# JiQi-da/Mixed-Graph-ADMM

Hardware: AMD Instinct MI355X
Metric: ADMM iters/sec x batch (sample-iterations/s) (higher is better)
Workload: dtype f32; 1 GPU; cfg2: PEMS04-shaped synthetic graph N=307 (path+chords, 340 edges), kNN k=4, T=24, t_in=12; batch_per_gpu=4096, global_batch=4096, ablation=None, graph=kNN-directed, max_cg_iter=100, parallelism=batch-sharded x1, no collective on the convergence path, final RCCL gather, all_finite=True

## Files before the change

mixed-graph-admm_amd/csrc/engine.h:

```cpp
#pragma once
#include <math.h>
#include <cmath>
#include <stdlib.h>
#include <string.h>

#include <algorithm>
#include <type_traits>

#include "common.h"
#include "cldr_tiles.h"
#include "stream_kernels.h"
#include "lds_args.h"
#include "lds_banks.h"

namespace {

struct LhsDef {
    int kind;
    int hth;
    double c1, c2;
};

enum VecId {
    V_XA, V_XB, V_ZUA, V_ZUB, V_ZDA, V_ZDB, V_PHIA, V_PHIB, V_GAM, V_GU, V_GD, V_Y, V_MASK,
    V_R, V_P, V_Q, V_AP, V_RHS, V_TMP, V_IO0, V_IO1, V_COUNT
};

constexpr int LAG = 2;
constexpr int NRED_MAX = 6;
constexpr int PROF_POOL = 32768;
constexpr int LDS_SETS = 3;
constexpr int LDS_NBOUND = 4;
constexpr int LDS_MAXJ_POOL = LDS_MAXJ;
constexpr int NACT_LOG = 1 << 16;

template <typename S>
// ... 21 lines not shown
    int* h_flag = nullptr;
    hipEvent_t ev_ring[LAG + 1] = {nullptr};
    int want_blocks = 2048;
    struct TileMetaDev { int R = 0; int GW = 0; int* tl_col = nullptr; float* tl_w = nullptr; int* halo = nullptr; int* h_rowptr = nullptr; int* h_col = nullptr; float* h_val = nullptr; };
    TileMetaDev tmeta[3];
    struct CldrDev {
        int state = 0, NT = 0;
        int *n0 = nullptr, *nC = nullptr, *rows = nullptr, *dcol = nullptr, *dcnt = nullptr, *tcol = nullptr, *tcnt = nullptr;
        float *dw = nullptr, *tw = nullptr;
    } cldr_dev;
    int use_fused = 1;
    int use_fold = 1;
    int use_fold_lu = 1;
    int sweep_rev = 1;
    int cldr_tile_major = 1;
    int cur_P = 0;
    int use_tile = 1;
    int64_t ws_bytes = 0;
    struct LdsPlan {
        bool ok = false;
        int G = 0, TPG = 0, TS = 0, nthreads = 0, block = 0, NR = 0, csr_ints = 0, maxt = 1024, sb = 0, uniform45 = 0, slots = 0;
        int tail_pairs = 0, lds_img0 = 0, lds_img_ints = 0;
        int off_rp_u = 0, off_rp_d = 0, off_en_u = 0, off_en_d = 0, off_lead_t = 0, off_tail_t = 0, off_diag = 0;
        size_t lds_bytes = 0;
    } lds;
    int* d_lds_csr = nullptr;
    double* d_m2 = nullptr;
    int lds_async = 1;
    int* d_stop = nullptr;
    double* d_ps_ring = nullptr;
    int* d_pstop = nullptr;
    double* d_ps_full = nullptr;
    size_t ps_full_elems = 0;
    int sp_B = 0;
    std::vector<double> sp_val[6];
    LdsSampleParams* d_sp = nullptr;
    std::vector<float*> lds_ring_extra;
    int64_t lds_instance = -1;
    int lds_chunk = LDS_MAXJ_POOL;
    hipStream_t st_side = nullptr;
    hipEvent_t ev_main[LDS_NBOUND] = {nullptr}, ev_side[LDS_NBOUND] = {nullptr};
    bool prof_on = false;
    std::vector<hipEvent_t> prof_ev;
    std::vector<int> prof_tag;
    std::vector<double> prof_lb;
    std::vector<int> prof_ref;
// ... 1299 lines not shown
        lds.maxt = (best == 12 && lds.block <= 640) ? 640 : 1024;
        lds.sb = (sb_env && ((best == 12 && lds.maxt == 640) || best == 8)) ? 1 : 0;
        const int NR = N + (lds.block - lds.nthreads);
        lds.NR = NR;
        lds.uniform45 = (!band && (best == 8 || best == 12) && !lds.sb && !getenv("MGADMM_LDS_RAGGED")) ? 1 : 0;
        for (int i = 0; i < N && lds.uniform45; ++i) {
            int ndiag = 0;
            for (int e = g->hWd.rowptr[i]; e < g->hWd.rowptr[i + 1]; ++e) ndiag += g->hWd.col[e] == i;
            if (g->hWu.rowptr[i + 1] - g->hWu.rowptr[i] != 4 || g->hWd.rowptr[i + 1] - g->hWd.rowptr[i] != 5 || ndiag != 1) lds.uniform45 = 0;
        }
        std::vector<float> diag_d(NR, 0.f), diag_t(NR, 0.f);
        auto strip_diag = [&](const HostCsr& h, std::vector<float>& dg) {
            HostCsr o;
            o.rowptr.push_back(0);
            for (int i = 0; i < N; ++i) {
                for (int e = h.rowptr[i]; e < h.rowptr[i + 1]; ++e) {
                    if (h.col[e] == i) dg[i] += h.val[e];
                    else { o.col.push_back(h.col[e]); o.val.push_back(h.val[e]); }
                }
                o.rowptr.push_back((int)o.col.size());
            }
            return o;
        };
        const HostCsr hWdT_off = band ? HostCsr() : strip_diag(g->hWdT, diag_t);
        int maxlen_t = 0;
        if (!band)
            for (int i = 0; i < N; ++i) maxlen_t = std::max(maxlen_t, hWdT_off.rowptr[i + 1] - hWdT_off.rowptr[i]);
        const int tp = band ? 0 : (std::max(0, maxlen_t - LDS_NLEAD) + 1) / 2;
        const int WT = LDS_NLEAD + 2 * tp;
        lds.tail_pairs = tp;
        const HostCsr hWd_tab = band ? HostCsr() : (lds.uniform45 ? strip_diag(g->hWd, diag_d) : g->hWd);
        auto with_ghosts = [&](const HostCsr& h, int fixed_len) {
            HostCsr o;
            o.rowptr.assign(h.rowptr.begin(), h.rowptr.begin() + N + 1);
            o.col = h.col; o.val = h.val;
            for (int r = N; r < NR; ++r) {
                for (int e = 0; e < fixed_len; ++e) { o.col.push_back(r); o.val.push_back(0.f); }
                o.rowptr.push_back((int)o.col.size());
            }
            return o;
        };
        const HostCsr hu = with_ghosts(g->hWu, lds.uniform45 ? 4 : 0);
        const HostCsr hd = band ? HostCsr() : with_ghosts(hWd_tab, lds.uniform45 ? 4 : 0);
        const int nu = hu.nnz(), nd = band ? 0 : hd.nnz();
        auto al4 = [](int v) { return (v + 3) & ~3; };
        int off = 0;
        lds.off_rp_u = off; off += NR + 1;
        lds.off_rp_d = off; off += NR + 1;
        off = al4(off);
        lds.off_en_u = off; off += 2 * nu;
        lds.off_en_d = off; off += 2 * nd;
        lds.off_lead_t = off; off += 2 * NR * LDS_NLEAD;
        off = al4(off);
        lds.off_tail_t = off; off += 2 * NR * 2 * tp + 4;
        const int tail_ints = off - lds.off_tail_t;
        lds.off_diag = off; off += 2 * NR;
        off += 8;
        lds.csr_ints = off;
        lds.lds_img0 = lds.uniform45 ? lds.off_tail_t : 0;
        lds.lds_img_ints = lds.uniform45 ? tail_ints : lds.off_diag;
        int ts = (T + 3) / 4 * 4;
        if (((ts / 4) & 1) == 0) ts += 4;
        auto bytes_for = [&](int stride, int slots) {
            const size_t LN = (size_t)NR * stride;
            return sizeof(float) * ((lds.sb ? 1 : 2) * LN + ((4 - (LN & 3)) & 3) + 32 + 16 * 12 + (size_t)slots * 2 * lds.block * best)
                   + sizeof(int) * (size_t)lds.lds_img_ints;
        };
        if (bytes_for(ts, 0) > 160 * 1024) ts = T;
        lds.TS = ts;
        if (bytes_for(ts, 0) > 160 * 1024) { lds = LdsPlan(); return MGADMM_OK; }
        lds.slots = (lds.uniform45 && !getenv("MGADMM_LDS_NOSLOTS") && bytes_for(ts, 1) <= 160 * 1024) ? 1 : 0;
        lds.lds_bytes = bytes_for(ts, lds.slots);
        std::vector<int> img(off, 0);
        const bool bank_order = !band && best % 4 == 0 && ((lds.TS / 4) & 1) && !getenv("MGADMM_LDS_TABLE_ORDER");
        long search_steps = 4000;
        if (const char* e = getenv("MGADMM_LDS_BANK_SEARCH")) search_steps = atol(e);
        auto slot_order = [&](const HostCsr& h, ldsbank::Stream stream) {
            std::vector<int> order(h.nnz());
            for (int e = 0; e < h.nnz(); ++e) order[e] = e;
            if (!bank_order || h.nnz() == 0) return order;
// ... 9 lines not shown
                std::vector<int> pos(N);
                for (int i = 0; i < N; ++i) pos[i] = i;
                const ldsbank::Result r = ldsbank::improve_targeted(q, m, pos, search_steps);
                if (getenv("MGADMM_LDS_BANK_STATS"))
                    fprintf(stderr, "[mgadmm] lds bank search: stream %d, %d entries: %.0f -> %.0f conflict cycles per application (%ld steps)\n",
                            (int)stream, h.rowptr[N], r.before, r.after, r.moves);
            }
            for (int e = 0; e < h.rowptr[N]; ++e) order[e] = m.src[e];
            return order;
        };
        auto put_entry = [&](int at, int col, float w) {
            img[at] = col * lds.TS;
            memcpy(&img[at + 1], &w, 4);
        };
        auto put_csr = [&](const HostCsr& h, int off_rp, int off_en, ldsbank::Stream stream) {
            const std::vector<int> order = slot_order(h, stream);
            for (int i = 0; i <= NR; ++i) img[off_rp + i] = h.rowptr[i];
            for (int e = 0; e < h.nnz(); ++e) put_entry(off_en + 2 * e, h.col[order[e]], h.val[order[e]]);
        };
        const ldsbank::Stream fixed_or_pairs = lds.uniform45 ? ldsbank::FIXED : ldsbank::PAIRS;
        put_csr(hu, lds.off_rp_u, lds.off_en_u, fixed_or_pairs);
        if (!band) {
            put_csr(hd, lds.off_rp_d, lds.off_en_d, fixed_or_pairs);
            HostCsr ht;
            ht.rowptr.push_back(0);
            std::vector<int> from;
            for (int i = 0; i < N; ++i) {
                const int e0 = hWdT_off.rowptr[i], len = hWdT_off.rowptr[i + 1] - e0;
                for (int e = 0; e < WT; ++e) {
                    ht.col.push_back(e < len ? hWdT_off.col[e0 + e] : i);
                    ht.val.push_back(e < len ? hWdT_off.val[e0 + e] : 0.f);
                    from.push_back(e < len ? e0 + e : -1);
                }
                ht.rowptr.push_back((int)ht.col.size());
            }
            const std::vector<int> order = slot_order(ht, ldsbank::FIXED);
            for (int r = 0; r < NR; ++r)
                for (int e = 0; e < WT; ++e) {
                    const int at = e < LDS_NLEAD ? lds.off_lead_t + 2 * (r * LDS_NLEAD + e)
                                                 : lds.off_tail_t + 2 * (r * 2 * tp + (e - LDS_NLEAD));
                    if (r < N) put_entry(at, ht.col[order[r * WT + e]], ht.val[order[r * WT + e]]);
                    else put_entry(at, r, 0.f);
                }
            put_entry(lds.off_tail_t + 2 * NR * 2 * tp, 0, 0.f);
            put_entry(lds.off_tail_t + 2 * NR * 2 * tp + 2, 0, 0.f);
            memcpy(&img[lds.off_diag], diag_d.data(), sizeof(float) * NR);
            memcpy(&img[lds.off_diag + NR], diag_t.data(), sizeof(float) * NR);
        }
        MG_HIP(hipMalloc(&d_lds_csr, sizeof(int) * off));
        MG_HIP(hipMemcpy(d_lds_csr, img.data(), sizeof(int) * off, hipMemcpyHostToDevice));
        MG_HIP(hipMalloc(&d_m2, sizeof(double) * T * N * (1 + (size_t)(Bmax + 63) / 64)));
        MG_HIP(hipMalloc(&d_stop, sizeof(int)));
        MG_HIP(hipMemset(d_stop, 0, sizeof(int)));
        MG_HIP(hipMalloc(&d_ps_ring, sizeof(double) * LDS_SETS * LDS_MAXJ_POOL * MGADMM_NMETRIC * Bp_max));
        MG_HIP(hipMalloc(&d_pstop, sizeof(int) * (2 * (size_t)Bp_max + 1)));
        {
            int lo = 0, hi = 0;
            MG_HIP(hipDeviceGetStreamPriorityRange(&lo, &hi));
            if (const char* e = getenv("MGADMM_LDS_SIDE_PRIO")) lo = atoi(e) > 0 ? hi : lo;
            MG_HIP(hipStreamCreateWithPriority(&st_side, hipStreamNonBlocking, lo));
            for (auto& e : ev_main) MG_HIP(hipEventCreateWithFlags(&e, hipEventDisableTiming));
            for (auto& e : ev_side) MG_HIP(hipEventCreateWithFlags(&e, hipEventDisableTiming));
        }
        lds.ok = true;
        return MGADMM_OK;
    }

    int launch_lds(const LdsArgs& a, int B) {
        const bool timed = prof_open(0, 0.0);
        LdsLaunch L{lds.TPG, lds.maxt, lds.sb, lds.uniform45, lds.slots, lds.block, lds.lds_bytes, &lds_instance};
        const int rc = mg_lds_iteration(L, a, B, st);
        if (timed) prof_close();
        return rc;
    }

    int solve_lds(const void* y, const void* mask, int B, const void* x0, const mgadmm_state* state_in, void* x_out,
                  const mgadmm_state* state_out, mgadmm_history* hist) {
        if constexpr (!std::is_same<S, float>::value) {
            return MGADMM_ERR_UNSUPPORTED;
        } else {
            const int abl = p.ablation;
            const bool has_phi = (abl == MGADMM_ABL_NONE || abl == MGADMM_ABL_DGLR);
            const bool has_zd = (abl != MGADMM_ABL_DGLR);
            const int max_it = p.max_admm_iter;
            const bool record = p.record_cg_coeffs && hist && hist->cg_alpha && hist->cg_beta;
            const int Bp = (B + 63) / 64 * 64;
            const size_t TN = (size_t)T * N;
            if (hist && hist->metrics_per_sample) {
                size_t need = (size_t)max_it * MGADMM_NMETRIC * B;
// ... 26 lines not shown
            constexpr int NRING = (int)(sizeof(ring_ids) / sizeof(ring_ids[0]));
            const int J = sched == CHUNKS ? std::max(1, std::min(std::min(lds_chunk, LDS_MAXJ_POOL), max_it)) : 1;
            {
                const int need = LDS_SETS * (J - 1) + LDS_NBOUND - NRING;
                while ((int)lds_ring_extra.size() < need) {
                    float* b = nullptr;
                    MG_HIP(hipMalloc(&b, vec_elems * sizeof(S)));
                    lds_ring_extra.push_back(b);
                    ws_bytes += (int64_t)(vec_elems * sizeof(S));
                }
            }
            auto ring = [&](int j) -> float* { return j < NRING ? (float*)vec[ring_ids[j]] : lds_ring_extra[j - NRING]; };
            auto xbuf = [&](int k) -> float* {
                if (k == max_it) return xo_;
                if (sched != CHUNKS) return ring(k & 1);
                if (k % J == 0) return ring((k / J) % LDS_NBOUND);
                return ring(LDS_NBOUND + ((k / J) % LDS_SETS) * (J - 1) + (k % J - 1));
            };
            float *zu = vec[V_ZUA], *zd = vec[V_ZDA], *phi = vec[V_PHIA], *gam = vec[V_GAM], *gu = vec[V_GU], *gd = vec[V_GD];
            if (state_in) {
                const size_t nb = (size_t)B * TN * sizeof(float);
                if (x0 != nullptr && xbuf(0) != x0) MG_HIP(hipMemcpyAsync(xbuf(0), x0, nb, hipMemcpyDeviceToDevice, st));
                auto in = [&](float* dst, const void* src) {
                    return src == nullptr ? (int)MGADMM_OK : mg_lds_state_layout(true, T, N, lds.TPG, B, (const float*)src, dst, st);
                };
                MG_TRY(in(zu, state_in->zu));
                MG_TRY(in(gu, state_in->gamma_u));
                MG_TRY(in(zd, state_in->zd));
                MG_TRY(in(gd, state_in->gamma_d));
                MG_TRY(in(phi, state_in->phi));
                MG_TRY(in(gam, state_in->gamma));
            } else {
                float tm = 0, t2m = 0;
                for (int t = 0; t < p.t_in; ++t) { tm += (float)t; t2m += (float)t * (float)t; }
                tm /= (float)p.t_in;
                t2m /= (float)p.t_in;
                const float den = t2m - tm * tm;
                MG_TRY(mg_lds_init(mask != nullptr, T, p.t_in, N, lds.TPG, B, tm, den, (const float*)y, (const float*)mask, xbuf(0), zu, zd, gam, gu, gd,
                                   d_nonfinite, st));
            }
            LdsArgs a{};
            a.T = T; a.N = N; a.TN = (int)TN; a.TS = lds.TS; a.t_in = p.t_in; a.G = lds.G; a.B = B; a.Bp = Bp;
            a.nthreads = lds.nthreads; a.NR = lds.NR; a.tail_pairs = lds.tail_pairs;
            a.has_phi = has_phi; a.has_zd = has_zd;
            const LhsDef dx = lhs_def(MGADMM_LHS_X);
            a.lhsx_kind = dx.kind == 1 ? 1 : 0;
            a.cx1 = (float)dx.c1; a.cx2 = (float)dx.c2;
            a.band = g->mode == MGADMM_TEMPORAL_BAND; a.skip = g->skip;
            a.q1 = a.band ? 0 : g->q1;
            a.max_cg = p.max_cg_iter; a.record = record ? 1 : 0;
            a.rho = (float)p.rho; a.rho_u = (float)p.rho_u; a.rho_d = (float)p.rho_d;
            a.mu_u = (float)p.mu_u; a.mu_d1 = (float)p.mu_d1; a.mu_d2 = (float)p.mu_d2;
            a.cg_tol2 = p.cg_tol * p.cg_tol;
            a.csr = d_lds_csr; a.lds_img0 = lds.lds_img0; a.lds_img_ints = lds.lds_img_ints;
            a.off_rp_u = lds.off_rp_u; a.off_rp_d = lds.off_rp_d;
            a.off_en_u = lds.off_en_u; a.off_en_d = lds.off_en_d; a.off_lead_t = lds.off_lead_t; a.off_tail_t = lds.off_tail_t; a.off_diag = lds.off_diag;
            a.band_w = g->band_w;
            a.zu = zu; a.zd = zd; a.phi = phi; a.gam = gam; a.gu = gu; a.gd = gd;
            {
                const int ncu = dev_cus > 0 ? dev_cus : 256;
                int us = 48;
                if (const char* e = getenv("MGADMM_LDS_STAGGER_US")) us = atoi(e);
                a.stagger_wgs = ncu;
                a.stagger_ticks = (B >= 2 * ncu && us > 0) ? us * 100 : 0;
            }
            a.y = (const float*)y; a.mask = (const float*)mask;
            a.alpha_hist = record ? (float*)d_alpha_hist : nullptr; a.beta_hist = record ? (float*)d_beta_hist : nullptr;
            a.nonfinite = d_nonfinite;
            a.stop = sched == DEVSTOP ? d_stop : nullptr;
            if (sched == DEVSTOP) MG_HIP(hipMemsetAsync(d_stop, 0, sizeof(int), st));
            if (sched == CHUNKS && !ps_mode) MG_HIP(hipMemsetAsync(d_ps_ring, 0, sizeof(double) * LDS_SETS * J * MGADMM_NMETRIC * Bp, st));
            int* const d_pcount = d_pstop + Bp_max;
            if (ps_mode) {
                a.pstop = d_pstop; a.pstop_count = d_pcount; a.x_final = xo_; a.admm_tol = p.admm_tol;
            }
            if (sp_B > 0) a.sp = d_sp;
            auto all_stopped = [&](int c, bool* done) -> int {
                MG_HIP(hipMemcpyAsync(h_flag + 1 + c % (LAG + 1), d_pcount, sizeof(int), hipMemcpyDeviceToHost, st));
                MG_HIP(hipEventRecord(ev_ring[c % (LAG + 1)], st));
// ... 95 lines not shown
            }
            if (sched == DEVSTOP) {
                MG_HIP(hipMemcpyAsync(h_flag + 1, d_stop, sizeof(int), hipMemcpyDeviceToHost, st));
                MG_HIP(hipStreamSynchronize(st));
                const int sw = h_flag[1];
                if (sw > 0) n_done = sw;
                else if (sw < 0) { n_done = -sw; rc_final = MGADMM_ERR_NONFINITE; }
            }
            std::vector<int> nps;
            if (ps_mode) {
                int* const d_nps = d_pstop + Bp_max + 1;
                MG_TRY(mg_lds_ps_history(d_ps_full, d_pstop, n_done, max_it, B, Bp, d_nps, d_hist,
                                         (hist && hist->metrics_per_sample) ? d_hist_ps : nullptr, st));
                nps.resize(B);
                MG_HIP(hipMemcpyAsync(nps.data(), d_nps, sizeof(int) * B, hipMemcpyDeviceToHost, st));
                MG_HIP(hipStreamSynchronize(st));
                n_done = *std::max_element(nps.begin(), nps.end());
            }
            float* const xc = ps_mode ? xo_ : xbuf(n_done);
            if (xc != xo_)
                MG_HIP(hipMemcpyAsync(x_out, xc, (size_t)B * TN * sizeof(float), hipMemcpyDeviceToDevice, st));
            if (state_out) {
                auto out = [&](void* dst, const float* src) {
                    return dst == nullptr ? (int)MGADMM_OK : mg_lds_state_layout(false, T, N, lds.TPG, B, src, (float*)dst, st);
                };
                MG_TRY(out(state_out->zu, zu));
                MG_TRY(out(state_out->zd, zd));
                if (has_phi) {
                    MG_TRY(out(state_out->phi, phi));
                    MG_TRY(out(state_out->gamma, gam));
                }
                MG_TRY(out(state_out->gamma_u, gu));
                MG_TRY(out(state_out->gamma_d, gd));
            }
            return finish_history(hist, n_done, B, Bp, rc_final, ps_mode ? nps.data() : nullptr);
        }
    }

    int finish_history(mgadmm_history* hist, int n_done, int B, int Bp, int rc_final, const int* nps = nullptr) {
        if (hist) {
            hist->n_iters = n_done;
            if (hist->n_iters_per_sample)
                for (int b = 0; b < B; ++b) hist->n_iters_per_sample[b] = nps ? nps[b] : n_done;
            if (hist->metrics)
                MG_HIP(hipMemcpyAsync(hist->metrics, d_hist, sizeof(double) * (size_t)n_done * MGADMM_NMETRIC, hipMemcpyDeviceToHost, st));
            if (hist->delta_x_per_step && !nps)
                MG_HIP(hipMemcpyAsync(hist->delta_x_per_step, d_dxps, sizeof(double) * (size_t)n_done * T, hipMemcpyDeviceToHost, st));
// ... 33 lines not shown
```

mixed-graph-admm_amd/csrc/lds_args.h:

```cpp
#pragma once
#include <hip/hip_runtime.h>

constexpr int LDS_NLEAD = 5;
constexpr int LDS_MAXJ = 16;

struct LdsArgsCore {
    int T, N, TN, TS, t_in, G, B, Bp;
    int nthreads;
    int NR;
    int has_phi, has_zd, first;
    int J;
    int lhsx_kind;
    int band, skip, q1;
    int max_cg;
    int record;
    int stagger_wgs, stagger_ticks;
    int tail_pairs;
    float rho, rho_u, rho_d, mu_u, mu_d1, mu_d2;
    float cx1, cx2;
    double cg_tol2;
    const int* csr;
    int lds_img0, lds_img_ints;
    int off_rp_u, off_rp_d, off_en_u, off_en_d, off_lead_t, off_tail_t;
    int off_diag;
    const float* band_w;
    float *zu, *zd, *phi, *gam, *gu, *gd;
    const float* y;
    const float* mask;
    double* ps;
    int* cg_iters;
    float* alpha_hist;
    float* beta_hist;
    int* nonfinite;
    const int* stop;
};
struct LdsSampleParams {
    float rho, rho_u, rho_d, mu_u, mu_d1, mu_d2;
    float cx1, cx2;
};
struct LdsArgs : LdsArgsCore {
    float* xs[LDS_MAXJ + 1];
    int* pstop;
    int* pstop_count;
    float* x_final;
    double admm_tol;
    int it0;
    const LdsSampleParams* sp;
};

struct LdsLaunch {
    int tpg;
    int maxt;
    int sb;
    int uniform45;
    int slots;
    int block;
    size_t lds_bytes;
    int64_t* instance;
};

int mg_lds_iteration(const LdsLaunch& L, const LdsArgs& a, int B, hipStream_t st);
int mg_lds_iteration_ps(const LdsLaunch& L, const LdsArgs& a, int B, hipStream_t st);
int mg_lds_iteration_pp(const LdsLaunch& L, const LdsArgs& a, int B, hipStream_t st);
int mg_lds_init(bool masked, int T, int t_in, int N, int TPG, int B, float tm, float den, const float* y, const float* mask, float* x,
                float* zu, float* zd, float* gam, float* gu, float* gd, int* nonfinite, hipStream_t st);
int mg_lds_state_layout(bool to_thread_major, int T, int N, int TPG, int B, const float* src, float* dst, hipStream_t st);
int mg_lds_dxps(int T, int N, int B, const float* x, const float* xo, double* scratch, double* out, const int* stop, hipStream_t st);
int mg_lds_ps_history(const double* ps, const int* pstop, int n_it, int max_it, int B, int Bp, int* n_per_sample, double* metrics,
                      double* out_ps, hipStream_t st);
int mg_lds_stop_test(const double* metrics_row, const int* nonfinite, int has_phi, int has_zd, double tol, int it, int* stop, hipStream_t st);
```

mixed-graph-admm_amd/csrc/lds_kernels.h:

```cpp
#pragma once
#include "common.h"
#include "lds_args.h"



template <int CTRL, int ROW_MASK>
__device__ __forceinline__ float dpp_step(float v) {
    const int moved = __builtin_amdgcn_update_dpp(0, __float_as_int(v), CTRL, ROW_MASK, 0xf, false);
    return v + __int_as_float(moved);
}
__device__ __forceinline__ float wave_sum(float v) {
    v = dpp_step<0x111, 0xf>(v);
    v = dpp_step<0x112, 0xf>(v);
    v = dpp_step<0x114, 0xf>(v);
    v = dpp_step<0x118, 0xf>(v);
    asm("s_nop 1\n\tv_add_f32_dpp %0, %0, %0 row_bcast:15 row_mask:0xa bank_mask:0xf\n\t"
        "s_nop 1\n\tv_add_f32_dpp %0, %0, %0 row_bcast:31 row_mask:0xc bank_mask:0xf\n\ts_nop 1" : "+v"(v));
    return __int_as_float(__builtin_amdgcn_readlane(__float_as_int(v), 63));
}

struct BlockRed {
    float* red;
    int par;
    int lane, wave, nwaves;
// ... 187 lines not shown
        for (int k = 0; k < TPG; ++k) v[k] = p[k];
    }
}

__device__ __forceinline__ float rhs_half(float rho, float z, float g) { return __builtin_fmaf(rho, z, -g) * 0.5f; }
__device__ __forceinline__ float ldrt_operand(float rho, float phi, float gam) { return __builtin_fmaf(rho, phi, gam); }

template <int TPG, bool BAND, int NU = 0, int ND = 0, int TP = -1>
struct LdsCtx {
    int T, TS, N, t0, i, ig;
    bool active;
    float* P;
    float* Q;
    const i2v* en_u; const i2v* en_d;
    const i2v* lead_t;
    const i2v* tail_t;
    int u0, u1, d0, d1;
    int tail_pairs;
    unsigned so0;
    unsigned kN4[TPG];
    f2 wdiag;
    int skip, q1;
    const float* band_w;

    __device__ __forceinline__ unsigned glb0() const { return 4u * (unsigned)(t0 * N + ig); }
    __device__ __forceinline__ int own() const { return i * TS + t0; }

    static constexpr bool UNI = NU > 0 && ND > 0;
    static constexpr int NDO = ND > 0 ? ND - 1 : 0;
    struct Rows {
        i2v u[NU > 0 ? NU : 1];
        i2v d[NDO > 0 ? NDO : 1];
        i2v t[LDS_NLEAD];
    };
    __device__ __forceinline__ i2v reg_entry(i2v e, const float* IMG) const {
        i2v r;
        r.x = lds_addr(IMG) + 4 * (e.x + t0);
        r.y = e.y;
        return r;
    }
    template <int NE>
    __device__ __forceinline__ void load_rows(const i2v* EN, int e0, const float* IMG, i2v (&en)[NE]) const {
        i2v raw[NE];
#pragma unroll
        for (int u = 0; u < NE; ++u) raw[u] = EN[e0 + u];
#pragma unroll
        for (int u = 0; u < NE; ++u) en[u] = reg_entry(raw[u], IMG);
    }

    template <int NE>
    __device__ __forceinline__ void gather_regs(const i2v (&en)[NE], int delta, float (&acc)[TPG]) const {
#pragma unroll
// ... 10 lines not shown
            wacc<TPG>(en[NE - 1], va, acc);
        }
    }
    __device__ __forceinline__ void gather(const float* SRC, const i2v* EN, int e0, int e1, float (&acc)[TPG]) const {
        const float* base = SRC + t0;
        i2v na = EN[e0], nb = EN[e0 + 1];
        int e = e0;
        for (; e + 1 < e1; e += 2) {
            const i2v ea = na, eb = nb;
            float va[TPG], vb[TPG];
            lds_load<TPG>(base + ea.x, va);
            lds_load<TPG>(base + eb.x, vb);
            na = EN[e + 2];
            nb = EN[e + 3];
            wacc<TPG>(ea, va, acc);
            wacc<TPG>(eb, vb, acc);
        }
        if (e < e1) {
            float va[TPG];
            lds_load<TPG>(base + na.x, va);
            wacc<TPG>(na, va, acc);
        }
    }
    __device__ __forceinline__ void gather_tail(const float* SRC, float (&acc)[TPG]) const {
        const float* base = SRC + t0;
        if constexpr (TP >= 0) {
            const lds_i4* row = reinterpret_cast<const lds_i4*>(tail_t + (size_t)i * 2 * TP);
            lds_i4 e2[TP > 0 ? TP : 1];
#pragma unroll
            for (int j = 0; j < TP; ++j) e2[j] = row[j];
#pragma unroll
            for (int j = 0; j < TP; ++j) {
                float va[TPG], vb[TPG];
                lds_load<TPG>(base + e2[j].x, va);
                lds_load<TPG>(base + e2[j].z, vb);
                wacc<TPG>(e2[j].xy, va, acc);
                wacc<TPG>(e2[j].zw, vb, acc);
            }
        } else {
            const lds_i4* row = reinterpret_cast<const lds_i4*>(tail_t + (size_t)i * 2 * tail_pairs);
            lds_i4 nxt = row[0];
            for (int j = 0; j < tail_pairs; ++j) {
                const lds_i4 e2 = nxt;
                float va[TPG], vb[TPG];
                lds_load<TPG>(base + e2.x, va);
                lds_load<TPG>(base + e2.z, vb);
                nxt = row[j + 1];
                wacc<TPG>(e2.xy, va, acc);
                wacc<TPG>(e2.zw, vb, acc);
            }
        }
    }

    __device__ __forceinline__ void mul_wu(const float* SRC, float (&acc)[TPG], const Rows& R) const {
#pragma unroll
        for (int k = 0; k < TPG; ++k) acc[k] = 0.f;
        if constexpr (UNI) gather_regs<NU>(R.u, lds_addr(SRC) - lds_addr(P), acc);
        else gather(SRC, en_u, u0, u1, acc);
    }
    __device__ __forceinline__ void mul_wd(const float* SRC, float (&acc)[TPG], const Rows& R, const float* own_run = nullptr) const {
// ... 368 lines not shown
    float xc[TPG], vc[TPG];
#pragma unroll
    for (int k = 0; k < TPG; ++k) xc[k] = vc[k] = 0.f;
    for (int trip = 0; trip < J; ++trip) {
#if defined(__HIP_DEVICE_COMPILE__)
    asm volatile("" : "+s"(kp));
    asm volatile("" : "+v"(tid));
    asm volatile("" : "+s"(b));
    const LdsArgs __attribute__((address_space(4)))& a = *kp;
#else
    const LdsArgs& a = *kp;
#endif
    const bool first = a.first && trip == 0;
#ifdef MGADMM_PHASE_CLOCK
    unsigned long long stamps[MGADMM_NMETRIC];
#define MG_STAMP(m) do { asm volatile("s_waitcnt vmcnt(0) lgkmcnt(0)" ::: "memory"); stamps[m] = wall_clock64(); } while (0)
#else
#define MG_STAMP(m) do { } while (0)
#endif
    MG_STAMP(0);
    LdsCtx<TPG, BAND, NU, ND, TP> c;
    c.T = a.T; c.TS = a.TS; c.N = a.N;
    c.active = tid < a.nthreads;
    {
        const int g = c.active ? tid / a.N : 0;
        c.ig = c.active ? tid - g * a.N : 0;
        c.i = c.active ? c.ig : a.N + (tid - a.nthreads);
        c.t0 = g * TPG;
    }
    c.P = P; c.Q = Q;
    c.skip = a.skip; c.q1 = a.q1; c.band_w = a.band_w;
    c.tail_pairs = a.tail_pairs;
#pragma unroll
    for (int k = 0; k < TPG; ++k) { c.kN4[k] = 4u * (unsigned)k * (unsigned)a.N; MG_PIN_S(c.kN4[k]); }
    c.so0 = c.active ? 4u * TPG * (unsigned)tid : 0u;
    {
        const int* tab = ENTG ? a.csr : img - a.lds_img0;
        c.en_u = reinterpret_cast<const i2v*>(tab + a.off_en_u);
        c.en_d = reinterpret_cast<const i2v*>(tab + a.off_en_d);
        c.lead_t = reinterpret_cast<const i2v*>(tab + a.off_lead_t);
        c.tail_t = reinterpret_cast<const i2v*>(img - a.lds_img0 + a.off_tail_t);
    }
    c.wdiag = mk2(0.f, 0.f);
    if constexpr (!BAND) {
        const float* dg = reinterpret_cast<const float*>(a.csr + a.off_diag);
        c.wdiag = mk2(dg[c.i], dg[a.NR + c.i]);
    }
    constexpr bool UNI = NU > 0 && ND > 0;
    constexpr int NDO = ND > 0 ? ND - 1 : 0;
    typename LdsCtx<TPG, BAND, NU, ND, TP>::Rows R;
    auto fetch_u = [&]() {
        if constexpr (UNI) {
// ... 106 lines not shown
    }
    MG_STAMP(1);
    __syncthreads();
    c.u0 = c.u1 = c.d0 = c.d1 = 0;
    if constexpr (NU > 0) c.u0 = c.i * NU;
    else { c.u0 = img[a.off_rp_u - a.lds_img0 + c.i]; c.u1 = img[a.off_rp_u - a.lds_img0 + c.i + 1]; }
    if constexpr (!BAND) {
        if constexpr (ND > 0) c.d0 = c.i * NDO;
        else { c.d0 = img[a.off_rp_d - a.lds_img0 + c.i]; c.d1 = img[a.off_rp_d - a.lds_img0 + c.i + 1]; }
    }
    BlockRed br;
    br.red = red; br.par = 0; br.lane = tid & 63; br.wave = tid >> 6; br.nwaves = (nthr + 63) >> 6;
    auto mput = [&](int m, float val) {
        const float w = wave_sum(val);
        if (br.lane == 0) mred[br.wave * NMRED + m] = w;
    };

    auto refresh = [&]() {
        MG_PIN_V(tid);
        MG_PIN_V(c.i); MG_PIN_V(c.ig); MG_PIN_V(c.t0);
        c.active = tid < a.nthreads;
        c.so0 = c.active ? 4u * TPG * (unsigned)tid : 0u;
        br.lane = tid & 63; br.wave = tid >> 6;
    };

    if (has_phi && first) {
        float ph[TPG];
        c.template put<-1>(P, x);
        __syncthreads();
        c.op_ldr(P, x, ph, R);
        c.puts(phi, ph);
        float gq[TPG];
        request1s(gam, gq);
#pragma unroll
        for (int k = 0; k < TPG; ++k) v[k] = c.active ? ldrt_operand(rho, ph[k], gq[k]) : 0.f;
        __syncthreads();
    }
    fetch_d();

    float rhs[TPG];
    {
        float l[TPG];
#pragma unroll
        for (int k = 0; k < TPG; ++k) l[k] = 0.f;
        if (has_phi) {
            c.template put<+1>(P, v);
// ... 270 lines not shown
        };
        double pri = rnorm(MGADMM_M_PRI_ZU), dual = rnorm(MGADMM_M_DUAL_ZU);
        if (has_phi) { pri = fmax(pri, rnorm(MGADMM_M_PRI_PHI)); dual = fmax(dual, rnorm(MGADMM_M_DUAL_PHI)); }
        if (has_zd) { pri = fmax(pri, rnorm(MGADMM_M_PRI_ZD)); dual = fmax(dual, rnorm(MGADMM_M_DUAL_ZD)); }
        const double atol = a.admm_tol;
        if (pri < atol && dual < atol) {
            c.putg(a.x_final + sb, xc);
            if (tid == 0) {
                a.pstop[b] = a.it0 + trip + 1;
                atomicAdd(a.pstop_count, 1);
            }
            break;
        }
    }
    }
}

__host__ __device__ __forceinline__ int lds_state_index(int t, int i, int N, int TPG) { return ((t / TPG) * N + i) * TPG + t % TPG; }

template <bool MASKED>
__global__ __launch_bounds__(256) void k_init_lds(int T, int t_in, int N, int TPG, int B, float tm, float den, const float* __restrict__ y,
                                                  const float* __restrict__ mask, float* __restrict__ x, float* __restrict__ zu,
                                                  float* __restrict__ zd, float* __restrict__ gam, float* __restrict__ gu,
                                                  float* __restrict__ gd, int* __restrict__ nonfinite) {
#pragma clang fp contract(off)
    const int i = blockIdx.x * 256 + threadIdx.x;
    const int b = blockIdx.y;
    if (i >= N) return;
    const size_t sb = (size_t)b * T * N;
    float w, c0;
    const float* yb = MASKED ? y + sb : y + (size_t)b * t_in * N;
    const float* mb = MASKED ? mask + sb : nullptr;
    if (!MASKED) {
        float sy = 0.f, sty = 0.f;
        for (int t = 0; t < t_in; ++t) {
            const float v = yb[t * N + i];
            sy += v;
            sty += (float)t * v;
        }
        const float ym = sy / (float)t_in;
        w = (sty / (float)t_in - tm * ym) / den;
        c0 = ym - w * tm;
    } else {
        float n = 0, ts = 0, t2s = 0, ys = 0, tys = 0;
        for (int t = 0; t < T; ++t) {
            const float m = mb[t * N + i], v = yb[t * N + i];
            n += m; ts += (float)t * m; t2s += (float)(t * t) * m;
            ys += v * m; tys += (float)t * v * m;
        }
        const float tmean = ts / n, t2mean = t2s / n, ymean = ys / n, tymean = tys / n;
        float tm2 = tmean * tmean;
        asm volatile("" : "+v"(tm2));
        const float dn = t2mean - tm2;
        w = (tymean - tmean * ymean) / dn;
        c0 = ymean - w * tmean;
        if (!(fabsf(w) <= 3.0e38f) || !(fabsf(c0) <= 3.0e38f)) *nonfinite = 1;
    }
    auto value = [&](int t) {
        if (!MASKED) return (t < t_in) ? yb[t * N + i] : w * (float)t + c0;
        return (w * (float)t + c0) * (1.f - mb[t * N + i]) + yb[t * N + i];
    };
    for (int t0 = 0; t0 < T; t0 += TPG) {
        const size_t es = sb + (size_t)((t0 / TPG) * N + i) * TPG;
        if (TPG % 4 == 0) {
            for (int k = 0; k < TPG; k += 4) {
                lds_f4 q;
                q.x = value(t0 + k); q.y = value(t0 + k + 1); q.z = value(t0 + k + 2); q.w = value(t0 + k + 3);
                x[sb + (size_t)(t0 + k) * N + i] = q.x; x[sb + (size_t)(t0 + k + 1) * N + i] = q.y;
                x[sb + (size_t)(t0 + k + 2) * N + i] = q.z; x[sb + (size_t)(t0 + k + 3) * N + i] = q.w;
                *reinterpret_cast<lds_f4*>(zu + es + k) = q;
                *reinterpret_cast<lds_f4*>(zd + es + k) = q;
                lds_f4 c; c.x = c.y = c.z = c.w = 0.1f;
                *reinterpret_cast<lds_f4*>(gam + es + k) = c;
                *reinterpret_cast<lds_f4*>(gu + es + k) = c;
                *reinterpret_cast<lds_f4*>(gd + es + k) = c;
            }
        } else {
            for (int k = 0; k < TPG; ++k) {
                const float v = value(t0 + k);
                x[sb + (size_t)(t0 + k) * N + i] = v;
                zu[es + k] = v; zd[es + k] = v;
                gam[es + k] = 0.1f; gu[es + k] = 0.1f; gd[es + k] = 0.1f;
            }
        }
    }
}

template <bool TO_THREAD_MAJOR>
__global__ __launch_bounds__(256) void k_state_layout(int T, int N, int TPG, const float* __restrict__ src, float* __restrict__ dst) {
    const int e = blockIdx.x * 256 + threadIdx.x;
    if (e >= T * N) return;
    const size_t sb = (size_t)blockIdx.y * T * N;
    const int t = e / N, i = e - t * N;
    const int es = lds_state_index(t, i, N, TPG);
    if (TO_THREAD_MAJOR) dst[sb + es] = src[sb + e];
    else dst[sb + e] = src[sb + es];
}

static __global__ __launch_bounds__(256) void k_dxps_sm(int TN, int B, const float* __restrict__ x, const float* __restrict__ xo,
                                                 double* __restrict__ part, const int* __restrict__ stop) {
    const int e = blockIdx.x * 256 + threadIdx.x;
    if (e >= TN || (stop != nullptr && *stop != 0)) return;
    const int b0 = blockIdx.y * 64, b1 = min(B, b0 + 64);
    double s = 0.0;
    for (int b = b0; b < b1; ++b) s += (double)x[(size_t)b * TN + e] - (double)xo[(size_t)b * TN + e];
    part[(size_t)blockIdx.y * TN + e] = s;
}

static __global__ __launch_bounds__(64) void k_dxps_sm4(int TN, int B, const float* __restrict__ x, const float* __restrict__ xo,
                                                 double* __restrict__ part, const int* __restrict__ stop) {
    const int e = (blockIdx.x * 64 + threadIdx.x) * 4;
    if (e >= TN || (stop != nullptr && *stop != 0)) return;
    const int b0 = blockIdx.y * 64, b1 = min(B, b0 + 64);
    double s0 = 0.0, s1 = 0.0, s2 = 0.0, s3 = 0.0;
    int b = b0;
    for (; b + 4 <= b1; b += 4) {
        lds_f4 a[4], o[4];
// ... 100 lines not shown
```

mixed-graph-admm_amd/csrc/lds_launch.hip:

```cpp
#include "lds_dispatch.h"

int mg_lds_iteration(const LdsLaunch& L, const LdsArgs& a, int B, hipStream_t st) {
    if (a.sp != nullptr) return mg_lds_iteration_pp(L, a, B, st);
    return a.pstop != nullptr ? mg_lds_iteration_ps(L, a, B, st) : lds_dispatch(L, a, B, st);
}

int mg_lds_init(bool masked, int T, int t_in, int N, int TPG, int B, float tm, float den, const float* y, const float* mask, float* x,
                float* zu, float* zd, float* gam, float* gu, float* gd, int* nonfinite, hipStream_t st) {
    dim3 grid((N + 255) / 256, B);
    if (masked) hipLaunchKernelGGL((k_init_lds<true>), grid, dim3(256), 0, st, T, t_in, N, TPG, B, tm, den, y, mask, x, zu, zd, gam, gu, gd, nonfinite);
    else hipLaunchKernelGGL((k_init_lds<false>), grid, dim3(256), 0, st, T, t_in, N, TPG, B, tm, den, y, (const float*)nullptr, x, zu, zd, gam, gu, gd, nonfinite);
    MG_HIP(hipGetLastError());
    return MGADMM_OK;
}

int mg_lds_state_layout(bool to_thread_major, int T, int N, int TPG, int B, const float* src, float* dst, hipStream_t st) {
    dim3 grid((T * N + 255) / 256, B);
    if (to_thread_major) hipLaunchKernelGGL((k_state_layout<true>), grid, dim3(256), 0, st, T, N, TPG, src, dst);
    else hipLaunchKernelGGL((k_state_layout<false>), grid, dim3(256), 0, st, T, N, TPG, src, dst);
    MG_HIP(hipGetLastError());
    return MGADMM_OK;
}

int mg_lds_dxps(int T, int N, int B, const float* x, const float* xo, double* scratch, double* out, const int* stop, hipStream_t st) {
    const int TN = T * N, nsl = (B + 63) / 64;
    if (TN % 4 == 0 && ((uintptr_t)x % 16) == 0 && ((uintptr_t)xo % 16) == 0)
        hipLaunchKernelGGL(k_dxps_sm4, dim3((TN / 4 + 63) / 64, nsl), dim3(64), 0, st, TN, B, x, xo, scratch + TN, stop);
    else
        hipLaunchKernelGGL(k_dxps_sm, dim3((TN + 255) / 256, nsl), dim3(256), 0, st, TN, B, x, xo, scratch + TN, stop);
    hipLaunchKernelGGL(k_dxps_sm_mean, dim3((TN + 255) / 256), dim3(256), 0, st, TN, B, nsl, (const double*)(scratch + TN), scratch, stop);
    hipLaunchKernelGGL(k_dxps_sm_final, dim3(T), dim3(256), 0, st, T, N, (const double*)scratch, out, stop);
    MG_HIP(hipGetLastError());
    return MGADMM_OK;
}

int mg_lds_stop_test(const double* metrics_row, const int* nonfinite, int has_phi, int has_zd, double tol, int it, int* stop, hipStream_t st) {
    hipLaunchKernelGGL(k_lds_stop_test, dim3(1), dim3(64), 0, st, metrics_row, nonfinite, has_phi, has_zd, tol, it, stop);
    MG_HIP(hipGetLastError());
    return MGADMM_OK;
}

int mg_lds_ps_history(const double* ps, const int* pstop, int n_it, int max_it, int B, int Bp, int* n_per_sample, double* metrics,
// ... 6 lines not shown
```

Measured before the change: 2.848 million ADMM sample-iterations/s.

## Reorder graph rows by transpose tail class so waves skip empty tail pairs

Relabels graph nodes so rows are sorted by how many transposed-directed-graph tail pairs they need, and records a per-wave maximum degree packed into a 64-bit launch word. In the LDS kernel each wave reads its count and runs only the tail-pair gathers its rows need, instead of the worst-case count for every row. Init and state-layout kernels are updated to map nodes to the permuted rows, and the bank-conflict table ordering is rebuilt for the padded-per-limit table. The cost is an extra indirection for the thread's node index, more wave-uniform branching, and more code for the relabeled layout.

```diff
diff --git a/mixed-graph-admm_amd/csrc/engine.h b/mixed-graph-admm_amd/csrc/engine.h
--- a/mixed-graph-admm_amd/csrc/engine.h
+++ b/mixed-graph-admm_amd/csrc/engine.h
@@ -12,6 +12,7 @@
 #include "stream_kernels.h"
 #include "lds_args.h"
 #include "lds_banks.h"
+#include "lds_rows.h"
 
 namespace {
 
@@ -79,6 +80,9 @@
         int G = 0, TPG = 0, TS = 0, nthreads = 0, block = 0, NR = 0, csr_ints = 0, maxt = 1024, sb = 0, uniform45 = 0, slots = 0;
         int tail_pairs = 0, lds_img0 = 0, lds_img_ints = 0;
         int off_rp_u = 0, off_rp_d = 0, off_en_u = 0, off_en_d = 0, off_lead_t = 0, off_tail_t = 0, off_diag = 0;
+        int row_order = 0;
+        int off_node = 0, off_rown = 0;
+        uint64_t npos_word = 0;
         size_t lds_bytes = 0;
     } lds;
     int* d_lds_csr = nullptr;
@@ -1424,14 +1428,27 @@
             }
             return o;
         };
-        const HostCsr hWdT_off = band ? HostCsr() : strip_diag(g->hWdT, diag_t);
-        int maxlen_t = 0;
+        std::vector<int> deg_t(N, 0);
         if (!band)
-            for (int i = 0; i < N; ++i) maxlen_t = std::max(maxlen_t, hWdT_off.rowptr[i + 1] - hWdT_off.rowptr[i]);
+            for (int i = 0; i < N; ++i)
+                for (int e = g->hWdT.rowptr[i]; e < g->hWdT.rowptr[i + 1]; ++e) deg_t[i] += g->hWdT.col[e] != i;
+        const int maxlen_t = N > 0 ? *std::max_element(deg_t.begin(), deg_t.end()) : 0;
         const int tp = band ? 0 : (std::max(0, maxlen_t - LDS_NLEAD) + 1) / 2;
         const int WT = LDS_NLEAD + 2 * tp;
         lds.tail_pairs = tp;
-        const HostCsr hWd_tab = band ? HostCsr() : (lds.uniform45 ? strip_diag(g->hWd, diag_d) : g->hWd);
+        const char* ro_env = getenv("MGADMM_LDS_ROW_ORDER");
+        lds.row_order = (lds.uniform45 && tp <= 3) ? (ro_env ? std::max(0, std::min(atoi(ro_env), 2)) : (int)ldsrows::TAIL_CLASS) : 0;
+        const ldsrows::Plan rows = ldsrows::make_plan(deg_t, lds.G, WT, lds.row_order, LDS_NLEAD);
+        lds.npos_word = 0;
+        if (lds.uniform45 && tp <= 3 && !ldsrows::pack_npos(rows, &lds.npos_word)) {
+            mg_set_error("lds: row plan does not fit its launch word (%d waves)", (int)rows.npos.size());
+            return MGADMM_ERR_INVALID;
+        }
+        const HostCsr Wu = lds.row_order ? ldsrows::relabel(g->hWu, rows) : g->hWu;
+        const HostCsr Wd = lds.row_order ? ldsrows::relabel(g->hWd, rows) : g->hWd;
+        const HostCsr WdT = lds.row_order ? ldsrows::relabel(g->hWdT, rows) : g->hWdT;
+        const HostCsr hWdT_off = band ? HostCsr() : strip_diag(WdT, diag_t);
+        const HostCsr hWd_tab = band ? HostCsr() : (lds.uniform45 ? strip_diag(Wd, diag_d) : Wd);
         auto with_ghosts = [&](const HostCsr& h, int fixed_len) {
             HostCsr o;
             o.rowptr.assign(h.rowptr.begin(), h.rowptr.begin() + N + 1);
@@ -1442,7 +1459,7 @@
             }
             return o;
         };
-        const HostCsr hu = with_ghosts(g->hWu, lds.uniform45 ? 4 : 0);
+        const HostCsr hu = with_ghosts(Wu, lds.uniform45 ? 4 : 0);
         const HostCsr hd = band ? HostCsr() : with_ghosts(hWd_tab, lds.uniform45 ? 4 : 0);
         const int nu = hu.nnz(), nd = band ? 0 : hd.nnz();
         auto al4 = [](int v) { return (v + 3) & ~3; };
@@ -1458,6 +1475,8 @@
         const int tail_ints = off - lds.off_tail_t;
         lds.off_diag = off; off += 2 * NR;
         off += 8;
+        lds.off_node = off; off += NR;
+        lds.off_rown = off; off += N;
         lds.csr_ints = off;
         lds.lds_img0 = lds.uniform45 ? lds.off_tail_t : 0;
         lds.lds_img_ints = lds.uniform45 ? tail_ints : lds.off_diag;
@@ -1513,24 +1532,18 @@
         put_csr(hu, lds.off_rp_u, lds.off_en_u, fixed_or_pairs);
         if (!band) {
             put_csr(hd, lds.off_rp_d, lds.off_en_d, fixed_or_pairs);
-            HostCsr ht;
-            ht.rowptr.push_back(0);
-            std::vector<int> from;
-            for (int i = 0; i < N; ++i) {
-                const int e0 = hWdT_off.rowptr[i], len = hWdT_off.rowptr[i + 1] - e0;
-                for (int e = 0; e < WT; ++e) {
-                    ht.col.push_back(e < len ? hWdT_off.col[e0 + e] : i);
-                    ht.val.push_back(e < len ? hWdT_off.val[e0 + e] : 0.f);
-                    from.push_back(e < len ? e0 + e : -1);
-                }
-                ht.rowptr.push_back((int)ht.col.size());
-            }
-            const std::vector<int> order = slot_order(ht, ldsbank::FIXED);
+            ldsbank::Geometry q;
+            q.N = N; q.G = T / best; q.TPG = best; q.TS = lds.TS; q.nlead = LDS_NLEAD;
+            ldsbank::Result sr;
+            const ldsrows::Table ht = ldsrows::build_table(q, hWdT_off.rowptr, hWdT_off.col, hWdT_off.val, rows, WT, bank_order, search_steps, &sr);
+            if (bank_order && search_steps > 0 && getenv("MGADMM_LDS_BANK_STATS"))
+                fprintf(stderr, "[mgadmm] lds bank search: W_d^T table, %d entries: %.0f -> %.0f conflict cycles per application (%ld steps)\n",
+                        hWdT_off.rowptr[N], sr.before, sr.after, sr.moves);
             for (int r = 0; r < NR; ++r)
                 for (int e = 0; e < WT; ++e) {
                     const int at = e < LDS_NLEAD ? lds.off_lead_t + 2 * (r * LDS_NLEAD + e)
                                                  : lds.off_tail_t + 2 * (r * 2 * tp + (e - LDS_NLEAD));
-                    if (r < N) put_entry(at, ht.col[order[r * WT + e]], ht.val[order[r * WT + e]]);
+                    if (r < N) put_entry(at, ht.col[(size_t)r * WT + e], ht.val[(size_t)r * WT + e]);
                     else put_entry(at, r, 0.f);
                 }
             put_entry(lds.off_tail_t + 2 * NR * 2 * tp, 0, 0.f);
@@ -1538,6 +1551,7 @@
             memcpy(&img[lds.off_diag], diag_d.data(), sizeof(float) * NR);
             memcpy(&img[lds.off_diag + NR], diag_t.data(), sizeof(float) * NR);
         }
+        for (int r = 0; r < N; ++r) { img[lds.off_node + r] = rows.node_of_row[r]; img[lds.off_rown + r] = rows.row_of_node[r]; }
         MG_HIP(hipMalloc(&d_lds_csr, sizeof(int) * off));
         MG_HIP(hipMemcpy(d_lds_csr, img.data(), sizeof(int) * off, hipMemcpyHostToDevice));
         MG_HIP(hipMalloc(&d_m2, sizeof(double) * T * N * (1 + (size_t)(Bmax + 63) / 64)));
@@ -1556,6 +1570,8 @@
         lds.ok = true;
         return MGADMM_OK;
     }
+
+    const int* lds_row_of_node() const { return lds.row_order ? d_lds_csr + lds.off_rown : nullptr; }
 
     int launch_lds(const LdsArgs& a, int B) {
         const bool timed = prof_open(0, 0.0);
@@ -1628,7 +1644,7 @@
                 const size_t nb = (size_t)B * TN * sizeof(float);
                 if (x0 != nullptr && xbuf(0) != x0) MG_HIP(hipMemcpyAsync(xbuf(0), x0, nb, hipMemcpyDeviceToDevice, st));
                 auto in = [&](float* dst, const void* src) {
-                    return src == nullptr ? (int)MGADMM_OK : mg_lds_state_layout(true, T, N, lds.TPG, B, (const float*)src, dst, st);
+                    return src == nullptr ? (int)MGADMM_OK : mg_lds_state_layout(true, T, N, lds.TPG, B, (const float*)src, dst, lds_row_of_node(), st);
                 };
                 MG_TRY(in(zu, state_in->zu));
                 MG_TRY(in(gu, state_in->gamma_u));
@@ -1643,7 +1659,7 @@
                 t2m /= (float)p.t_in;
                 const float den = t2m - tm * tm;
                 MG_TRY(mg_lds_init(mask != nullptr, T, p.t_in, N, lds.TPG, B, tm, den, (const float*)y, (const float*)mask, xbuf(0), zu, zd, gam, gu, gd,
-                                   d_nonfinite, st));
+                                   d_nonfinite, lds_row_of_node(), st));
             }
             LdsArgs a{};
             a.T = T; a.N = N; a.TN = (int)TN; a.TS = lds.TS; a.t_in = p.t_in; a.G = lds.G; a.B = B; a.Bp = Bp;
@@ -1661,6 +1677,7 @@
             a.csr = d_lds_csr; a.lds_img0 = lds.lds_img0; a.lds_img_ints = lds.lds_img_ints;
             a.off_rp_u = lds.off_rp_u; a.off_rp_d = lds.off_rp_d;
             a.off_en_u = lds.off_en_u; a.off_en_d = lds.off_en_d; a.off_lead_t = lds.off_lead_t; a.off_tail_t = lds.off_tail_t; a.off_diag = lds.off_diag;
+            a.npos = lds.npos_word; a.off_node = lds.off_node;
             a.band_w = g->band_w;
             a.zu = zu; a.zd = zd; a.phi = phi; a.gam = gam; a.gu = gu; a.gd = gd;
             {
@@ -1802,7 +1819,7 @@
                 MG_HIP(hipMemcpyAsync(x_out, xc, (size_t)B * TN * sizeof(float), hipMemcpyDeviceToDevice, st));
             if (state_out) {
                 auto out = [&](void* dst, const float* src) {
-                    return dst == nullptr ? (int)MGADMM_OK : mg_lds_state_layout(false, T, N, lds.TPG, B, src, (float*)dst, st);
+                    return dst == nullptr ? (int)MGADMM_OK : mg_lds_state_layout(false, T, N, lds.TPG, B, src, (float*)dst, lds_row_of_node(), st);
                 };
                 MG_TRY(out(state_out->zu, zu));
                 MG_TRY(out(state_out->zd, zd));
diff --git a/mixed-graph-admm_amd/csrc/lds_args.h b/mixed-graph-admm_amd/csrc/lds_args.h
--- a/mixed-graph-admm_amd/csrc/lds_args.h
+++ b/mixed-graph-admm_amd/csrc/lds_args.h
@@ -46,6 +46,8 @@
     double admm_tol;
     int it0;
     const LdsSampleParams* sp;
+    unsigned long long npos;
+    int off_node;
 };
 
 struct LdsLaunch {
@@ -63,8 +65,8 @@
 int mg_lds_iteration_ps(const LdsLaunch& L, const LdsArgs& a, int B, hipStream_t st);
 int mg_lds_iteration_pp(const LdsLaunch& L, const LdsArgs& a, int B, hipStream_t st);
 int mg_lds_init(bool masked, int T, int t_in, int N, int TPG, int B, float tm, float den, const float* y, const float* mask, float* x,
-                float* zu, float* zd, float* gam, float* gu, float* gd, int* nonfinite, hipStream_t st);
-int mg_lds_state_layout(bool to_thread_major, int T, int N, int TPG, int B, const float* src, float* dst, hipStream_t st);
+                float* zu, float* zd, float* gam, float* gu, float* gd, int* nonfinite, const int* row_of_node, hipStream_t st);
+int mg_lds_state_layout(bool to_thread_major, int T, int N, int TPG, int B, const float* src, float* dst, const int* row_of_node, hipStream_t st);
 int mg_lds_dxps(int T, int N, int B, const float* x, const float* xo, double* scratch, double* out, const int* stop, hipStream_t st);
 int mg_lds_ps_history(const double* ps, const int* pstop, int n_it, int max_it, int B, int Bp, int* n_per_sample, double* metrics,
                       double* out_ps, hipStream_t st);
diff --git a/mixed-graph-admm_amd/csrc/lds_kernels.h b/mixed-graph-admm_amd/csrc/lds_kernels.h
--- a/mixed-graph-admm_amd/csrc/lds_kernels.h
+++ b/mixed-graph-admm_amd/csrc/lds_kernels.h
@@ -233,12 +233,14 @@
     f2 wdiag;
     int skip, q1;
     const float* band_w;
+    int npos;
 
     __device__ __forceinline__ unsigned glb0() const { return 4u * (unsigned)(t0 * N + ig); }
     __device__ __forceinline__ int own() const { return i * TS + t0; }
 
     static constexpr bool UNI = NU > 0 && ND > 0;
     static constexpr int NDO = ND > 0 ? ND - 1 : 0;
+    static constexpr bool ROWPLAN = UNI && TP >= 0;
     struct Rows {
         i2v u[NU > 0 ? NU : 1];
         i2v d[NDO > 0 ? NDO : 1];
@@ -295,20 +297,30 @@
             wacc<TPG>(na, va, acc);
         }
     }
+    template <int NP>
+    __device__ __forceinline__ void tail_pairs_n(const lds_i4* row, const float* base, float (&acc)[TPG]) const {
+        lds_i4 e2[NP > 0 ? NP : 1];
+#pragma unroll
+        for (int j = 0; j < NP; ++j) e2[j] = row[j];
+#pragma unroll
+        for (int j = 0; j < NP; ++j) {
+            float va[TPG], vb[TPG];
+            lds_load<TPG>(base + e2[j].x, va);
+            lds_load<TPG>(base + e2[j].z, vb);
+            wacc<TPG>(e2[j].xy, va, acc);
+            wacc<TPG>(e2[j].zw, vb, acc);
+        }
+    }
     __device__ __forceinline__ void gather_tail(const float* SRC, float (&acc)[TPG]) const {
         const float* base = SRC + t0;
         if constexpr (TP >= 0) {
             const lds_i4* row = reinterpret_cast<const lds_i4*>(tail_t + (size_t)i * 2 * TP);
-            lds_i4 e2[TP > 0 ? TP : 1];
-#pragma unroll
-            for (int j = 0; j < TP; ++j) e2[j] = row[j];
-#pragma unroll
-            for (int j = 0; j < TP; ++j) {
-                float va[TPG], vb[TPG];
-                lds_load<TPG>(base + e2[j].x, va);
-                lds_load<TPG>(base + e2[j].z, vb);
-                wacc<TPG>(e2[j].xy, va, acc);
-                wacc<TPG>(e2[j].zw, vb, acc);
+            if constexpr (ROWPLAN && TP > 0) {
+                if constexpr (TP >= 3) if (npos > LDS_NLEAD + 4) { tail_pairs_n<3>(row, base, acc); return; }
+                if constexpr (TP >= 2) if (npos > LDS_NLEAD + 2) { tail_pairs_n<2>(row, base, acc); return; }
+                if (npos > LDS_NLEAD) tail_pairs_n<1>(row, base, acc);
+            } else {
+                tail_pairs_n<TP>(row, base, acc);
             }
         } else {
             const lds_i4* row = reinterpret_cast<const lds_i4*>(tail_t + (size_t)i * 2 * tail_pairs);
@@ -723,12 +735,24 @@
     LdsCtx<TPG, BAND, NU, ND, TP> c;
     c.T = a.T; c.TS = a.TS; c.N = a.N;
     c.active = tid < a.nthreads;
+    constexpr bool ROWPLAN = LdsCtx<TPG, BAND, NU, ND, TP>::ROWPLAN;
+    auto wave_npos = [&]() {
+        int n = 0;
+        if constexpr (ROWPLAN) {
+            n = (int)((a.npos >> (4 * __builtin_amdgcn_readfirstlane(tid >> 6))) & 15);
+            MG_PIN_S(n);
+        }
+        return n;
+    };
     {
         const int g = c.active ? tid / a.N : 0;
-        c.ig = c.active ? tid - g * a.N : 0;
-        c.i = c.active ? c.ig : a.N + (tid - a.nthreads);
+        const int r = c.active ? tid - g * a.N : 0;
+        c.i = c.active ? r : a.N + (tid - a.nthreads);
+        if constexpr (ROWPLAN) c.ig = a.csr[a.off_node + c.i];
+        else c.ig = r;
         c.t0 = g * TPG;
     }
+    c.npos = wave_npos();
     c.P = P; c.Q = Q;
     c.skip = a.skip; c.q1 = a.q1; c.band_w = a.band_w;
     c.tail_pairs = a.tail_pairs;
@@ -881,6 +905,7 @@
         c.active = tid < a.nthreads;
         c.so0 = c.active ? 4u * TPG * (unsigned)tid : 0u;
         br.lane = tid & 63; br.wave = tid >> 6;
+        c.npos = wave_npos();
     };
 
     if (has_phi && first) {
@@ -1197,7 +1222,8 @@
 __global__ __launch_bounds__(256) void k_init_lds(int T, int t_in, int N, int TPG, int B, float tm, float den, const float* __restrict__ y,
                                                   const float* __restrict__ mask, float* __restrict__ x, float* __restrict__ zu,
                                                   float* __restrict__ zd, float* __restrict__ gam, float* __restrict__ gu,
-                                                  float* __restrict__ gd, int* __restrict__ nonfinite) {
+                                                  float* __restrict__ gd, int* __restrict__ nonfinite,
+                                                  const int* __restrict__ row_of_node) {
 #pragma clang fp contract(off)
     const int i = blockIdx.x * 256 + threadIdx.x;
     const int b = blockIdx.y;
@@ -1235,8 +1261,9 @@
         if (!MASKED) return (t < t_in) ? yb[t * N + i] : w * (float)t + c0;
         return (w * (float)t + c0) * (1.f - mb[t * N + i]) + yb[t * N + i];
     };
+    const int ir = row_of_node ? row_of_node[i] : i;
     for (int t0 = 0; t0 < T; t0 += TPG) {
-        const size_t es = sb + (size_t)((t0 / TPG) * N + i) * TPG;
+        const size_t es = sb + (size_t)((t0 / TPG) * N + ir) * TPG;
         if (TPG % 4 == 0) {
             for (int k = 0; k < TPG; k += 4) {
                 lds_f4 q;
@@ -1262,12 +1289,13 @@
 }
 
 template <bool TO_THREAD_MAJOR>
-__global__ __launch_bounds__(256) void k_state_layout(int T, int N, int TPG, const float* __restrict__ src, float* __restrict__ dst) {
+__global__ __launch_bounds__(256) void k_state_layout(int T, int N, int TPG, const float* __restrict__ src, float* __restrict__ dst,
+                                                      const int* __restrict__ row_of_node) {
     const int e = blockIdx.x * 256 + threadIdx.x;
     if (e >= T * N) return;
     const size_t sb = (size_t)blockIdx.y * T * N;
     const int t = e / N, i = e - t * N;
-    const int es = lds_state_index(t, i, N, TPG);
+    const int es = lds_state_index(t, row_of_node ? row_of_node[i] : i, N, TPG);
     if (TO_THREAD_MAJOR) dst[sb + es] = src[sb + e];
     else dst[sb + e] = src[sb + es];
 }
diff --git a/mixed-graph-admm_amd/csrc/lds_launch.hip b/mixed-graph-admm_amd/csrc/lds_launch.hip
--- a/mixed-graph-admm_amd/csrc/lds_launch.hip
+++ b/mixed-graph-admm_amd/csrc/lds_launch.hip
@@ -6,18 +6,18 @@
 }
 
 int mg_lds_init(bool masked, int T, int t_in, int N, int TPG, int B, float tm, float den, const float* y, const float* mask, float* x,
-                float* zu, float* zd, float* gam, float* gu, float* gd, int* nonfinite, hipStream_t st) {
+                float* zu, float* zd, float* gam, float* gu, float* gd, int* nonfinite, const int* row_of_node, hipStream_t st) {
     dim3 grid((N + 255) / 256, B);
-    if (masked) hipLaunchKernelGGL((k_init_lds<true>), grid, dim3(256), 0, st, T, t_in, N, TPG, B, tm, den, y, mask, x, zu, zd, gam, gu, gd, nonfinite);
-    else hipLaunchKernelGGL((k_init_lds<false>), grid, dim3(256), 0, st, T, t_in, N, TPG, B, tm, den, y, (const float*)nullptr, x, zu, zd, gam, gu, gd, nonfinite);
+    if (masked) hipLaunchKernelGGL((k_init_lds<true>), grid, dim3(256), 0, st, T, t_in, N, TPG, B, tm, den, y, mask, x, zu, zd, gam, gu, gd, nonfinite, row_of_node);
+    else hipLaunchKernelGGL((k_init_lds<false>), grid, dim3(256), 0, st, T, t_in, N, TPG, B, tm, den, y, (const float*)nullptr, x, zu, zd, gam, gu, gd, nonfinite, row_of_node);
     MG_HIP(hipGetLastError());
     return MGADMM_OK;
 }
 
-int mg_lds_state_layout(bool to_thread_major, int T, int N, int TPG, int B, const float* src, float* dst, hipStream_t st) {
+int mg_lds_state_layout(bool to_thread_major, int T, int N, int TPG, int B, const float* src, float* dst, const int* row_of_node, hipStream_t st) {
     dim3 grid((T * N + 255) / 256, B);
-    if (to_thread_major) hipLaunchKernelGGL((k_state_layout<true>), grid, dim3(256), 0, st, T, N, TPG, src, dst);
-    else hipLaunchKernelGGL((k_state_layout<false>), grid, dim3(256), 0, st, T, N, TPG, src, dst);
+    if (to_thread_major) hipLaunchKernelGGL((k_state_layout<true>), grid, dim3(256), 0, st, T, N, TPG, src, dst, row_of_node);
+    else hipLaunchKernelGGL((k_state_layout<false>), grid, dim3(256), 0, st, T, N, TPG, src, dst, row_of_node);
     MG_HIP(hipGetLastError());
     return MGADMM_OK;
 }
diff --git a/mixed-graph-admm_amd/csrc/lds_rows.h b/mixed-graph-admm_amd/csrc/lds_rows.h
--- /dev/null
+++ b/mixed-graph-admm_amd/csrc/lds_rows.h
@@ -0,0 +1,114 @@
+#pragma once
+#include <algorithm>
+#include <cstdint>
+#include <numeric>
+#include <vector>
+
+#include "lds_banks.h"
+
+namespace ldsrows {
+
+struct Plan {
+    std::vector<int> node_of_row, row_of_node;
+    std::vector<int> npos;
+    std::vector<int> lim;
+};
+
+enum Order { NODE = 0, IN_DEGREE = 1, TAIL_CLASS = 2 };
+
+inline Plan make_plan(const std::vector<int>& deg, int G, int width, int order, int nlead = 0) {
+    const int N = (int)deg.size();
+    const int nw = (N * G + 63) / 64;
+    const bool reorder = order != NODE;
+    Plan p;
+    p.node_of_row.resize(N);
+    std::iota(p.node_of_row.begin(), p.node_of_row.end(), 0);
+    auto key = [&](int i) { return order == TAIL_CLASS ? (std::max(0, deg[i] - nlead) + 1) / 2 : deg[i]; };
+    if (reorder) std::stable_sort(p.node_of_row.begin(), p.node_of_row.end(), [&](int a, int b) { return key(a) > key(b); });
+    p.row_of_node.resize(N);
+    for (int r = 0; r < N; ++r) p.row_of_node[p.node_of_row[r]] = r;
+    p.npos.assign(nw, reorder ? 0 : width);
+    if (reorder)
+        for (int tid = 0; tid < N * G; ++tid) p.npos[tid / 64] = std::max(p.npos[tid / 64], deg[p.node_of_row[tid % N]]);
+    p.lim.assign(N, width);
+    for (int tid = 0; tid < N * G; ++tid) p.lim[tid % N] = std::min(p.lim[tid % N], p.npos[tid / 64]);
+    return p;
+}
+
+inline bool pack_npos(const Plan& p, uint64_t* word) {
+    if (p.npos.size() > 16) return false;
+    uint64_t v = 0;
+    for (size_t w = 0; w < p.npos.size(); ++w) {
+        if (p.npos[w] < 0 || p.npos[w] > 15) return false;
+        v |= (uint64_t)p.npos[w] << (4 * w);
+    }
+    *word = v;
+    return true;
+}
+
+template <typename Csr>
+inline Csr relabel(const Csr& h, const Plan& p) {
+    const int N = (int)p.node_of_row.size();
+    Csr o = h;
+    o.rowptr.assign(1, 0);
+    o.col.clear();
+    o.val.clear();
+    for (int r = 0; r < N; ++r) {
+        const int i = p.node_of_row[r];
+        for (int e = h.rowptr[i]; e < h.rowptr[i + 1]; ++e) {
+            o.col.push_back(p.row_of_node[h.col[e]]);
+            o.val.push_back(h.val[e]);
+        }
+        o.rowptr.push_back((int)o.col.size());
+    }
+    return o;
+}
+
+struct Table {
+    std::vector<int> col, from;
+    std::vector<float> val;
+};
+inline Table build_table(const ldsbank::Geometry& q, const std::vector<int>& rowptr, const std::vector<int>& col, const std::vector<float>& val,
+                         const Plan& p, int width, bool bank_order, long search_steps, ldsbank::Result* stats = nullptr) {
+    const int N = q.N;
+    ldsbank::Mat m;
+    m.stream = ldsbank::FIXED;
+    m.rowptr.push_back(0);
+    for (int r = 0; r < N; ++r) {
+        const int e0 = rowptr[r], len = rowptr[r + 1] - e0;
+        const int w = std::max(len, std::min(p.lim[r], width));
+        for (int e = 0; e < w; ++e) {
+            m.col.push_back(e < len ? col[e0 + e] : r);
+            m.src.push_back(e < len ? e0 + e : -1);
+        }
+        m.rowptr.push_back((int)m.col.size());
+    }
+    if (bank_order && !m.col.empty()) {
+        std::vector<int> src0 = m.src;
+        for (size_t e = 0; e < m.src.size(); ++e) m.src[e] = (int)e;
+        ldsbank::greedy_order(q, m);
+        if (search_steps > 0) {
+            std::vector<int> pos(N);
+            std::iota(pos.begin(), pos.end(), 0);
+            const ldsbank::Result r = ldsbank::improve_targeted(q, m, pos, search_steps);
+            if (stats) *stats = r;
+        }
+        for (size_t e = 0; e < m.src.size(); ++e) m.src[e] = src0[m.src[e]];
+    }
+    Table t;
+    t.col.resize((size_t)N * width);
+    t.from.assign((size_t)N * width, -1);
+    t.val.assign((size_t)N * width, 0.f);
+    for (int r = 0; r < N; ++r) {
+        const int e0 = m.rowptr[r], w = m.rowptr[r + 1] - e0;
+        for (int e = 0; e < width; ++e) {
+            const int s = e < w ? m.src[e0 + e] : -1;
+            t.col[(size_t)r * width + e] = s >= 0 ? col[s] : r;
+            t.val[(size_t)r * width + e] = s >= 0 ? val[s] : 0.f;
+            t.from[(size_t)r * width + e] = s;
+        }
+    }
+    return t;
+}
+
+}
```

Result: faster. 3.008 million ADMM sample-iterations/s (median of 6 runs) (+5.6%).
